# rg2/DeepFluoroLabeling-IPCAI2020

Hardware: AMD Instinct MI355X
Metric: train images/sec, paper U-Net (depth 6, wf 5, BN, strided-conv down, seg + 14-landmark heads), 1x192x192 (8x-downsampled 184x184 padded) (higher is better)
Workload: dtype bf16 (bf16 activations, activation gradients and GEMM weight copies in HBM; bf16 MFMA, fp32 accumulate, BatchNorm statistics, losses, weight gradients and master weights); 1 GPU; BASELINE configs[1]: 8x-downsampled, seg + 14-landmark heat-map dual head, batch 16 per GPU, Dice+NCC loss, SGD nesterov; global_batch=16, image=1x192x192, parallelism=dp1, math=bf16s, optimizer=dfl_amd.SGD(momentum 0.9, nesterov, wd 1e-4)

## Files before the change

### deepfluorolabeling-ipcai2020_amd/_native.py

```python
import ctypes as C
import os

from . import _cabi

_HERE = os.path.dirname(os.path.abspath(__file__))
LIB_PATH = os.environ.get('DFL_LIB_OVERRIDE') or os.path.join(_HERE, 'lib', 'libdfl_hip.so')

i32, i64, f32 = C.c_int32, C.c_int64, C.c_float
fp = C.c_void_p

_CONSTANTS, _STRUCTS, _FUNCTIONS = _cabi.load()
globals().update({name[len('DFL_'):]: value for name, value in _CONSTANTS.items()})
globals().update({cls.__name__: cls for cls in _STRUCTS.values()})
EXPORTS = list(_FUNCTIONS)

CONV_CFG_LATENCY = 39

_KIND_OF = {ConvArgs: OP_CONV, WgradArgs: OP_WGRAD, SumPartialsArgs: OP_SUM_PARTIALS, PackArgs: OP_PACK,
            BnFinalizeArgs: OP_BN_FINALIZE, BnEvalArgs: OP_BN_EVAL, ColstatsArgs: OP_COLSTATS,
            BnBwdFinalizeArgs: OP_BN_BWD_FINALIZE, BnReluBwdArgs: OP_BN_RELU_BWD,
            ReducePartialsArgs: OP_REDUCE_PARTIALS, AffineCopyArgs: OP_AFFINE_COPY, HeadFwdArgs: OP_HEAD_FWD,
            HeadBwdArgs: OP_HEAD_BWD, MemsetArgs: OP_MEMSET, ReduceBatchArgs: OP_REDUCE_BATCH, BnLiveArgs: OP_BN_FINALIZE_LIVE, BnBwdLiveArgs: OP_BN_BWD_FINALIZE_LIVE,
            ConvPairArgs: OP_CONV_PAIR}

# ... 170 lines not shown
        n = len(self.structs) - start if count is None else count
        h = C.c_void_p()
        check(lib().dfl_graph_capture(C.addressof(self._ops) + start * C.sizeof(Op), n, stream, C.addressof(h)),
              'dfl_graph_capture')
        return Graph(h.value, self)

    MIN_GRAPH_OPS = 2

    def graph_chunks(self, stream, start=0, count=None):
        n = len(self.structs) - start if count is None else count
        key = (start, n)
        chunks = self._chunks.get(key)
        if chunks is None:
            chunks, i, end = [], start, start + n
            while i < end:
                plain = self.kinds[i] in (OP_RECORD, OP_WAIT) or self.streams[i] != 0 or self.volatile[i]
                j = i + 1
                while j < end and (self.kinds[j] in (OP_RECORD, OP_WAIT) or self.streams[j] != 0 or self.volatile[j]) == plain:
                    j += 1
                if not plain and j - i >= self.MIN_GRAPH_OPS:
                    chunks.append((i, j - i, self.capture(stream, i, j - i)))
                else:
                    chunks.append((i, j - i, None))
                i = j
            self._chunks[key] = chunks
        return chunks

    def run_graphed(self, stream, start=0, count=None):
        if not self.structs:
            return
        for first, cnt, graph in self.graph_chunks(stream, start, count):
            if graph is not None:
                graph.launch(stream)
            else:
                self.run(stream, first, cnt)
# ... 10 lines not shown
```

### deepfluorolabeling-ipcai2020_amd/csrc/api.hip

```cpp
#include <stdlib.h>
#include <string.h>

#include <mutex>
#include <vector>

#include "common.h"

namespace dfl {
static thread_local char g_err[512] = "";

void set_error(const char* fmt, ...) {
  va_list ap;
  va_start(ap, fmt);
  vsnprintf(g_err, sizeof(g_err), fmt, ap);
  va_end(ap);
}
}

namespace dfl {
static std::mutex g_sync_mu;
static hipStream_t g_side[DFL_MAX_SIDE_STREAMS] = {nullptr};
static std::vector<hipEvent_t> g_events;

static hipStream_t pick_stream(int id, hipStream_t main) {
// ... 59 lines not shown
      (int)sizeof(dfl_preproc_projs_args),   (int)sizeof(dfl_preproc_segs_args),
      (int)sizeof(dfl_restore_labels_args), (int)sizeof(dfl_sim_prepare_args),  (int)sizeof(dfl_sim_gradncc_args),
      (int)sizeof(dfl_expose_args),     (int)sizeof(dfl_sim_patch_prepare_args), (int)sizeof(dfl_sim_patch_gradncc_args),
      (int)sizeof(dfl_raster_mesh),    (int)sizeof(dfl_raster_args),
      (int)sizeof(dfl_sim_gradncc_bwd_args), (int)sizeof(dfl_sim_patch_weights_args), (int)sizeof(dfl_sim_patch_eval_args),
      (int)sizeof(dfl_drr_pose_grad_args),
      (int)sizeof(dfl_sim_bank_gradncc_args), (int)sizeof(dfl_sim_bank_gradncc_bwd_args), (int)sizeof(dfl_sim_patch_bank_gradncc_args),
      (int)sizeof(dfl_drr_object),     (int)sizeof(dfl_drr_args),
      (int)sizeof(dfl_optim_pack_args)};
  if (which < 0 || which >= (int)(sizeof(sizes) / sizeof(sizes[0]))) return -1;
  return sizes[which];
}

static int exec_one(const dfl_op* ops, int i, dfl_stream_t stream, bool serial);

extern "C" int dfl_exec(const dfl_op* ops, int32_t n_ops, dfl_stream_t stream) {
  if (ops == nullptr || n_ops < 0) {
    dfl::set_error("dfl_exec: bad arguments");
    return DFL_ERR_INVALID_ARG;
  }
  for (int i = 0; i < n_ops; ++i) {
    int rc = exec_one(ops, i, stream, false);
    if (rc != DFL_OK) return rc;
  }
  return DFL_OK;
}

extern "C" int dfl_exec_timed(const dfl_op* ops, int32_t n_ops, dfl_stream_t stream, float* ms_out) {
  if (ops == nullptr || n_ops <= 0 || ms_out == nullptr) {
    dfl::set_error("dfl_exec_timed: bad arguments");
    return DFL_ERR_INVALID_ARG;
  }
  hipStream_t s = static_cast<hipStream_t>(stream);
  hipEvent_t* ev = new hipEvent_t[n_ops + 1];
  for (int i = 0; i <= n_ops; ++i) (void)hipEventCreate(&ev[i]);
  int rc = DFL_OK;
  (void)hipEventRecord(ev[0], s);
  int done = 0;
  for (int i = 0; i < n_ops; ++i) {
    rc = exec_one(ops, i, stream, true);
// ... 25 lines not shown
  }
  *graph_out = nullptr;
  (void)stream;
  hipStream_t s = nullptr;
  hipError_t err = hipStreamCreateWithFlags(&s, hipStreamNonBlocking);
  if (err != hipSuccess) {
    dfl::set_error("dfl_graph_capture: hipStreamCreateWithFlags: %s", hipGetErrorString(err));
    return DFL_ERR_LAUNCH;
  }
  err = hipStreamBeginCapture(s, hipStreamCaptureModeThreadLocal);
  if (err != hipSuccess) {
    (void)hipStreamDestroy(s);
    dfl::set_error("dfl_graph_capture: hipStreamBeginCapture: %s", hipGetErrorString(err));
    return DFL_ERR_LAUNCH;
  }
  int rc = DFL_OK;
  for (int i = 0; i < n_ops && rc == DFL_OK; ++i) rc = exec_one(ops, i, static_cast<dfl_stream_t>(s), true);
  hipGraph_t g = nullptr;
  err = hipStreamEndCapture(s, &g);
  (void)hipStreamDestroy(s);
  if (rc != DFL_OK) {
    if (g != nullptr) (void)hipGraphDestroy(g);
    return rc;
  }
  if (err != hipSuccess || g == nullptr) {
    dfl::set_error("dfl_graph_capture: hipStreamEndCapture: %s", hipGetErrorString(err));
    return DFL_ERR_LAUNCH;
  }
  hipGraphExec_t e = nullptr;
  err = hipGraphInstantiate(&e, g, nullptr, nullptr, 0);
  if (err != hipSuccess) {
    (void)hipGraphDestroy(g);
// ... 140 lines not shown
```

### deepfluorolabeling-ipcai2020_amd/plan.py

```python
import ctypes as C
import os

import numpy as np
import torch

from . import _native as nat
from ._native import (ConvArgs, WgradArgs, PackJob, BnFinalizeArgs, ColstatsArgs, BnBwdFinalizeArgs, BnReluBwdArgs,
                      AffineCopyArgs, PoolArgs, HeadFwdArgs, HeadBwdArgs, PackArgs, BnEvalArgs, UpsampleArgs, BnLiveJob, BnLiveArgs,
                      BnBwdLiveJob, BnBwdLiveArgs, MemsetArgs, ReduceJob, ReduceBatchArgs, Program)

BN_EPS = 1.0e-5
BN_MOMENTUM = 0.1


class Act:
    __slots__ = ('t', 'ptr', 'ld', 'N', 'H', 'W', 'C', 'esz')

    def __init__(self, t, ptr, ld, N, H, W, C, esz=4):
        self.t, self.ptr, self.ld, self.N, self.H, self.W, self.C, self.esz = t, ptr, ld, N, H, W, C, esz

    @property
    def M(self):
        return self.N * self.H * self.W

    @property
    def bf16(self):
        return int(self.esz == 2)

    def chan_slice(self, c0, c):
        return Act(self.t, self.ptr + self.esz * c0, self.ld, self.N, self.H, self.W, c, self.esz)


class PlanError(RuntimeError):
    pass


KEEP_GRADS = False


class _Layer:
    __slots__ = ('w', 'wname', 'relu', 'inp', 'gin', 'inp_aff', 'r', 'bn', 'live_bwd')

    def __init__(self, w, wname, relu, inp, gin, inp_aff, r, bn, live_bwd):
        self.w, self.wname, self.relu, self.inp, self.gin, self.inp_aff = w, wname, relu, inp, gin, inp_aff
        self.r, self.bn, self.live_bwd = r, bn, live_bwd


class _Block:
    __slots__ = ('prefix', 'xin', 'out', 'convs', 'rw', 'last_r', 'last_live')
# ... 2 lines not shown
        self.prefix, self.xin, self.out = prefix, xin, out
        self.convs = []
        self.rw = None
        self.last_r = None
        self.last_live = False


class UNetPlan:
    PACK_TILED = os.environ.get('DFL_PACK_TILED', '1') != '0'
    FUSE_BRB = os.environ.get('DFL_FUSE_BRB', '1') != '0'
    FUSE_DOWN_STATS = os.environ.get('DFL_FUSE_DOWN_STATS', '1') != '0'
    FLUSH_BYTES = int(float(os.environ.get('DFL_FLUSH_MB', '16')) * (1 << 20))
    DPRE_OUT_BYTES = int(float(os.environ.get('DFL_DPRE_OUT_MB', '12')) * (1 << 20))
    LIVE_BN = os.environ.get('DFL_LIVE_BN', '1') != '0'
    LIVE_HEAD = os.environ.get('DFL_LIVE_HEAD', '1') != '0'
    BN_R = nat.BN_R

    def __init__(self, cfg, params, buffers, N, H, W, training, need_grad, device, input_grad=False):
        self.cfg = cfg
        self.P = params
        self.Bf = buffers
        self.N, self.H, self.W = N, H, W
        self.training = training
        self.need_grad = need_grad
        self.input_grad = bool(input_grad and need_grad)
        self.dx_in = None
        self.dev = device
        self.lib = nat.lib()
        self._keep = []
        self.fwd = Program()
# ... 8 lines not shown
        self._red_bytes = 0
        self._red_flushes = []
        self.partial_sum_bytes = 0
        self._tiled_host = self._tiled_index = None
        self.math = self.lib.dfl_get_math_mode()
        self.bf16 = self.math == 4
        self.adt = torch.bfloat16 if self.bf16 else torch.float32
        self.aesz = 2 if self.bf16 else 4
        self._packed_split = {}
        self.relu_out = {}
        self._tot_fwd, self._tot_bwd, self._live_jobs, self._live_bwd_pending = [None, 0], [None, 0], [], []
        self.dbg = {}
        self.keep_grads = bool(KEEP_GRADS)
        self.pool_in = {}
        self._latency_form = int(not training and not need_grad and os.environ.get('DFL_PLAN_LATENCY_FORM', '1') != '0')
        self._build()

    def _new(self, nelem, dtype=torch.float32):
        t = torch.empty(max(int(nelem), 1), dtype=dtype, device=self.dev)
        self._keep.append(t)
        return t

    def _const(self, n, value):
        key = ('const', int(n), float(value))
        t = self._scratch.get(key)
        if t is None:
            t = torch.full((int(n),), float(value), dtype=torch.float32, device=self.dev)
            self._keep.append(t)
            self._scratch[key] = t
        return t

    def _act(self, N, H, W, C):
        t = self._new(N * H * W * C, self.adt)
        return Act(t, t.data_ptr(), C, N, H, W, C, self.aesz)

    def _scratch_act(self, key, N, H, W, C):
        need = N * H * W * C
        t = self._scratch.get(key)
        if t is None or t.numel() < need:
            raise PlanError('scratch %s not sized' % key)
        if self.keep_grads:
            return self._act(N, H, W, C)
        return Act(t, t.data_ptr(), C, N, H, W, C, self.aesz)

    def _pack(self, w, kind, flip=0):
        A, B, KH, KW = w.shape
        Cc = KH * KW
        K = {1: Cc * B, 2: Cc * A, 3: A}[kind]
        N = {1: A, 2: B, 3: Cc * B}[kind]
        cin = B if kind == 1 else A
        if self.bf16 and cin % 16 == 0:
            dst = self._new((K + 15) // 16 * N * 16, torch.bfloat16)
            self._packed_split[dst.data_ptr()] = 2
            self._pack_jobs.append((w, dst, A, B, Cc, kind, flip, 2))
            return dst
        dst = self._new((K + 3) // 4 * N * 4)
        split = int(self.math in (1, 3) and cin % 16 == 0)
        self._packed_split[dst.data_ptr()] = split
# ... 11 lines not shown

    def _pack_convT_fwd(self, w):
        return self._pack(w, 3)

    def _pack_convT_dgrad(self, w):
        return self._pack(w, 1)

    @staticmethod
    def _set_pack_job(a, job):
        src, dst, A, B, Cc, kind, flip, split = job
        a.src, a.dst, a.A, a.B, a.C, a.kind, a.flip, a.split = src.data_ptr(), dst.data_ptr(), A, B, Cc, kind, flip, split

    def _upload(self, arr):
        t = torch.from_numpy(np.frombuffer(bytes(arr), dtype=np.uint8).copy()).to(self.dev)
        self._keep.append(t)
        return t.data_ptr()

    def _finish_pack(self):
        self.pack = Program()
        self.pack.extend(self._prep)
        if not self._pack_jobs:
            return
        if self.PACK_TILED:
            self._finish_pack_tiled()
        else:
            self._add_pack_launch(self._pack_jobs)

    def _add_pack_launch(self, jobs):
        arr = (PackJob * len(jobs))()
        for a, job in zip(arr, jobs):
            self._set_pack_job(a, job)
# ... 82 lines not shown
            a.splits = sp
            a.partial = self._shared_scratch('conv_partial', sp * M * Ntot).data_ptr()
        partials = None
        if stat_totals is not None:
            a.stat_totals = stat_totals
            if stat_other is not None:
                a.stat_other, a.ldso = stat_other.ptr, stat_other.ld
            partials = ('live', stat_totals)
        elif stats:
            gm = nat.check(self.lib.dfl_conv_grid_m(C.addressof(a)), 'dfl_conv_grid_m')
            partials = self._new(gm * 2 * Ntot)
            a.stat_partials = partials.data_ptr()
            if stat_other is not None:
                a.stat_other, a.ldso = stat_other.ptr, stat_other.ld
            partials = (partials, 4 * gm if scatter else gm)
        prog.add(a)
        return partials

    def _wgrad(self, prog, g, d, dw, KH, KW, stride, pad, Hout, Wout, in_aff=None, d_split=0, brb=None,
               bias_out=None, bias_plain=False):
        a = WgradArgs()
        a.d_split = d_split
        a.g_bf16, a.d_bf16 = g.bf16, d.bf16
        a.g, a.d, a.dw = g.ptr, d.ptr, dw.data_ptr()
        if in_aff is not None:
            a.in_scale, a.in_shift = in_aff[0].data_ptr(), in_aff[1].data_ptr()
        a.N, a.Hin, a.Win, a.Cg, a.ldg = g.N, g.H, g.W, g.C, g.ld
        a.KH, a.KW, a.stride, a.pad = KH, KW, stride, pad
        a.Hout, a.Wout, a.Cm, a.ldd = Hout, Wout, d.C, d.ld
        if brb is not None:
            r_act, coef = brb
# ... 4 lines not shown
            else:
                a.coef = nat.ptr(coef)
        a.splits = 1
        s = nat.check(self.lib.dfl_wgrad_suggest_splits(C.addressof(a)), 'dfl_wgrad_suggest_splits')
        a.splits = s
        bias_job = None
        if (brb is not None or bias_plain) and bias_out is not None:
            bpart = self._new(s * d.C)
            a.bias_partial = bpart.data_ptr()
            bias_job = (bpart.data_ptr(), bias_out.data_ptr(), d.C, d.C, s, 1)
        n = d.C * g.C * KH * KW
        if s > 1:
            big = 4 * n >= self.FLUSH_BYTES
            part = self._shared_scratch('wg_partial', s * n) if big else self._new(s * n)
            a.partial = part.data_ptr()
        prog.add(a)
        if bias_job is not None:
            self._red_pending.append(bias_job)
            self._red_bytes += 4 * d.C
        if s > 1:
            self._defer_sum(prog, part.data_ptr(), dw.data_ptr(), n, n, s, KH * KW)

    def _defer_sum(self, prog, src, dst, n, stride, count, T=1):
        self._red_pending.append((src, dst, n, stride, count, T))
        self._red_bytes += 4 * n
        self._maybe_flush(prog)

    def _maybe_flush(self, prog):
        if self._red_bytes >= self.FLUSH_BYTES:
            self._flush_sums(prog)

    def _flush_sums(self, prog):
        self._flush_live_bwd(prog)
        jobs = self._red_pending
        if not jobs:
            return
        arr = (ReduceJob * len(jobs))()
        blocks = 0
        for a, (src, dst, n, stride, count, T) in zip(arr, jobs):
            a.src, a.dst, a.n, a.stride, a.count, a.first_block, a.T = src, dst, n, stride, count, blocks, T
            blocks += nat.check(self.lib.dfl_reduce_job_blocks(n, count), 'dfl_reduce_job_blocks')
        self._red_flushes.append((len(prog.structs), [j[1] for j in jobs]))
        self.partial_sum_bytes += sum(4 * n * count for (_, _, n, _, count, _) in jobs)
        prog.add(ReduceBatchArgs(jobs_dev=self._upload(arr), njobs=len(jobs), total_blocks=blocks))
        self._red_pending, self._red_bytes = [], 0

    def _dz_for(self, g, N, H, W, Cc, fused):
        key = 'dpre0' if fused and g.t is self._scratch.get('dz') else 'dz'
        return self._scratch_act(key, N, H, W, Cc)

    def _bn_totals(self, Cc, bwd=False):
        need = self.BN_R * 2 * Cc
        ar = self._tot_bwd if bwd else self._tot_fwd
        if ar[0] is None:
            ar[0] = self._new(sum(self.chans) * self.bd * 2 * self.BN_R * 2, torch.float64)
        assert ar[1] + need <= ar[0].numel()
        ptr = ar[0].data_ptr() + 8 * ar[1]
        ar[1] += need
        return ptr

    def _flush_live_bwd(self, prog):
        jobs = self._live_bwd_pending
        if not jobs:
            return
        arr = (BnBwdLiveJob * len(jobs))()
        for a, j in zip(arr, jobs):
            a.totals, a.save_mean, a.save_invstd = j['tot'], j['mean'].data_ptr(), j['invstd'].data_ptr()
            a.dgamma, a.dbeta, a.sum_out, a.C = j['dgamma'].data_ptr(), j['dbeta'].data_ptr(), nat.ptr(j['sum_out']), j['C']
        dsts = [j[k].data_ptr() for j in jobs for k in ('dgamma', 'dbeta', 'sum_out') if j[k] is not None]
        self._red_flushes.append((len(prog.structs), dsts))
        prog.add(BnBwdLiveArgs(jobs_dev=self._upload(arr), njobs=len(jobs), max_C=max(j['C'] for j in jobs)))
        self._live_bwd_pending = []

    def _finish_live_bn(self):
        jobs = self._live_jobs
        if not jobs:
            return
        arr = (BnLiveJob * len(jobs))()
        for a, j in zip(arr, jobs):
            a.totals, a.gamma, a.beta = j['totals'], j['gamma'].data_ptr(), j['beta'].data_ptr()
            a.running_mean = self.Bf[j['bname'] + '.running_mean'].data_ptr()
            a.running_var = self.Bf[j['bname'] + '.running_var'].data_ptr()
            a.num_batches_tracked = self.Bf[j['bname'] + '.num_batches_tracked'].data_ptr()
            a.scale, a.shift, a.save_mean, a.save_invstd = (j[k].data_ptr() for k in ('scale', 'shift', 'mean', 'invstd'))
            a.count, a.C, a.eps, a.momentum = j['count'], j['C'], BN_EPS, BN_MOMENTUM
        self.fwd.add(BnLiveArgs(jobs_dev=self._upload(arr), njobs=len(jobs), max_C=max(j['C'] for j in jobs)))
        self.fwd.insert(0, MemsetArgs(ptr=self._tot_fwd[0].data_ptr(), bytes=8 * self._tot_fwd[1]))

    def _shared_scratch(self, key, nelem):
        t = self._scratch.get(key)
        if t is None or t.numel() < nelem:
            t = self._new(nelem)
            self._scratch[key] = t
        return t

    def _colsum(self, prog, a, out):
        nb = self.lib.dfl_rowblock_count(a.M, a.C)
        part = self._new(nb * 2 * a.C)
        prog.add(ColstatsArgs(a=a.ptr, b=None, partials=part.data_ptr(), M=a.M, C=a.C, lda=a.ld, ldb=0, nblocks=nb,
                              bf16=a.bf16))
        self._defer_sum(prog, part.data_ptr(), out.data_ptr(), a.C, 2 * a.C, nb)

    _WRAP = ((-1, 0, 1), (0, 1, None), (0, None, 1))

    def _wrap_regions(self, H, W):
        out = []
        for sy, dy, h in ((H - 1, 0, 1), (0, 1, H), (0, H + 1, 1)):
            for sx, dx, w in ((W - 1, 0, 1), (0, 1, W), (0, W + 1, 1)):
                out.append((sy, sx, dy, dx, h, w))
        return out

    def _wrap_pad(self, prog, x):
        n = x.N * (x.H + 2) * (x.W + 2) * x.C
        t = self._new(n, torch.bfloat16 if x.esz == 2 else torch.float32)
        xp = Act(t, t.data_ptr(), x.C, x.N, x.H + 2, x.W + 2, x.C, x.esz)
        for sy, sx, dy, dx, h, w in self._wrap_regions(x.H, x.W):
            prog.add(AffineCopyArgs(x=x.ptr, y=xp.ptr, N=x.N, H=h, W=w, C=x.C, ldx=x.ld, xH=x.H, xW=x.W, xoy=sy, xox=sx,
                                    ldy=xp.ld, yH=xp.H, yW=xp.W, yoy=dy, yox=dx, bf16=x.bf16))
        return xp

    def _wrap_fold(self, prog, dxp, dx, accumulate=0):
        regs = self._wrap_regions(dx.H, dx.W)
        regs.sort(key=lambda r: 0 if (r[4] == dx.H and r[5] == dx.W) else 1)
        for i, (sy, sx, dy, dx_, h, w) in enumerate(regs):
            prog.add(AffineCopyArgs(x=dxp.ptr, y=dx.ptr, N=dx.N, H=h, W=w, C=dx.C, ldx=dxp.ld, xH=dxp.H, xW=dxp.W, xoy=dy, xox=dx_,
                                    ldy=dx.ld, yH=dx.H, yW=dx.W, yoy=sy, yox=sx, accumulate=(accumulate if i == 0 else 1), bf16=dx.bf16))

    def _framed_grad(self, like):
        n = like.N * (like.H + 2) * (like.W + 2) * like.C
        t = self._new(n, self.adt)
        return Act(t, t.data_ptr(), like.C, like.N, like.H + 2, like.W + 2, like.C, self.aesz)

    def _build(self):
        self._levels()
        self._alloc_buffers()
        self._down_forward()
        self._up_forward()
        self._finish_live_bn()
        self._heads_forward()
        if self.need_grad:
# ... 362 lines not shown
        if mfma_head and live_r is not None:
            tot = self._bn_totals(Fx, bwd=True)
            hb.stat_other, hb.ldso, hb.stat_totals = live_r.ptr, live_r.ld, tot
            live = ('live', tot)
        if fused_head:
            part = self._new(4096 * nat.check(self.lib.dfl_head_wgrad_blocks(M_), 'dfl_head_wgrad_blocks'))
            hb.wg_partial = part.data_ptr()
            hb.dw_seg = gs.data_ptr()
            if nl > 0:
                hb.dw_l1 = g1.data_ptr()
                if w2 is not None:
                    hb.dw_l2 = g2.data_ptr()
        else:
            scratch = self._new(M_ * sld)
            hb.scratch = scratch.data_ptr()
        bwd.add(hb, volatile=True)
        if not fused_head:
            off = [self.lib.dfl_head_scratch_off_for(Fx, NC, nm, nl, k) for k in range(5)]
            sact = lambda o, c: Act(scratch, scratch.data_ptr() + 4 * o, sld, N, H_, W_, c)
            self._wgrad(bwd, sact(off[0], Fx), sact(off[1], NC), gs, 1, 1, 1, 0, H_, W_)
            if nl > 0:
                self._wgrad(bwd, sact(off[0], Fx + NC), sact(off[2], nm), g1, 1, 1, 1, 0, H_, W_)
                if w2 is not None:
                    self._wgrad(bwd, sact(off[3], nm), sact(off[4], nl), g2, 1, 1, 1, 0, H_, W_)
        return hb, dx, live

    def _lands_block_backward(self, dfeat, dfeat_a):
        N, G, bwd, u = self.N, self.G, self.bwd, self.feat
        F, Fh = u.C, dfeat.C
        hl, wl = self.heat_hw
        if self.split_heads:
            dout = dfeat_a
            src_u = dfeat.chan_slice(0, F)
            bwd.add(AffineCopyArgs(x=src_u.ptr, y=dout.ptr, N=N, H=hl, W=wl, C=F, ldx=src_u.ld, xH=hl, xW=wl, ldy=dout.ld,
                                   yH=u.H, yW=u.W, yoy=(u.H - hl) // 2, yox=(u.W - wl) // 2, accumulate=1, bf16=dout.bf16))
        else:
            dout = dfeat.chan_slice(0, F)
        d = dfeat.chan_slice(F, Fh - F)
        for j in reversed(range(len(self.lb_layers))):
            src, dst, wname, bname, gin, ho_, wo_ = self.lb_layers[j]
            self._colsum(bwd, d, G[bname])
            self._wgrad(bwd, gin, d, G[wname], 3, 3, 1, 0 if self.circular else self.pad, ho_, wo_)
            wd = self._pack_conv_dgrad(self.P[wname])
            tgt = dout if j == 0 else self._act(N, src.H, src.W, Fh - F)
            if self.circular:
                dzp = self._framed_grad(src)
                self._conv(bwd, d, wd, dzp, 3, 3, 1, 2, src.C)
                self._wrap_fold(bwd, dzp, tgt, accumulate=1 if j == 0 else 0)
            else:
# ... 10 lines not shown
            Ci = self.chans[i]
            st = self._block_backward(rec['blk'], dout, self.dcat[i], fused_in=sums, dxin_stats=True)
            dy = self.dcat[i].chan_slice(0, Ci)
            uin = rec['u']
            bias_name = rec['name'] + ('.up.1.bias' if self.upsample else '.up.bias')
            if st is not None:
                self._defer_sum(bwd, st[0].data_ptr(), G[bias_name].data_ptr(), Ci, 4 * Ci, st[1])
            else:
                self._colsum(bwd, dy, G[bias_name])
            du = self._act(N, uin.H, uin.W, uin.C)
            self.dbg['du:%d' % j] = du
            consumer = self._up[j - 1]['blk'] if j > 0 else self._down[-1]['blk']
            r_last = consumer.last_r
            if self.upsample:
                dylow = self._act(N, uin.H, uin.W, Ci)
                bwd.add(UpsampleArgs(x=dylow.ptr, y=dy.ptr, N=N, H=uin.H, W=uin.W, C=Ci, ldx=dylow.ld, ldy=dy.ld, bf16=dy.bf16),
                        nat.OP_UPSAMPLE_BWD)
                self._wgrad(bwd, uin, dylow, G[rec['name'] + '.up.1.weight'], 1, 1, 1, 0, uin.H, uin.W)
                sums = self._conv(bwd, dylow, self._pack_conv_dgrad(rec['w']), du, 1, 1, 1, 0, uin.C,
                                  stats=r_last is not None, stat_other=r_last,
                                  stat_totals=self._bn_totals(uin.C, bwd=True) if (r_last is not None and consumer.last_live) else None)
            else:
                self._wgrad(bwd, dy, uin, G[rec['name'] + '.up.weight'], 2, 2, 2, 0, uin.H, uin.W)
                wd = self._pack_convT_dgrad(rec['w'])
                sums = self._conv(bwd, dy, wd, du, 2, 2, 2, 0, uin.C, stats=r_last is not None, stat_other=r_last,
                                  stat_totals=self._bn_totals(uin.C, bwd=True) if (r_last is not None and consumer.last_live) else None)
            dout = du
        return dout, sums

    def _down_backward(self, dout, sums):
        N, G, bwd = self.N, self.G, self.bwd
        dnxt = dnxt_sums = None
        for i in reversed(range(self.depth)):
            rec = self._down[i]
            blk = rec['blk']
            out = blk.out
            Ci = self.chans[i]
            if i != self.depth - 1:
                sums = None
                if self.direct_bridge[i]:
                    dout = self.dcat[i].chan_slice(Ci, Ci)
                else:
                    dout = self._act(N, out.H, out.W, Ci)
                    oy, ox, ch, cw = rec['crop']
                    src = self.dcat[i].chan_slice(Ci, Ci)
                    bwd.add(MemsetArgs(ptr=dout.ptr, bytes=dout.esz * dout.M * Ci))
                    bwd.add(AffineCopyArgs(x=src.ptr, y=dout.ptr, N=N, H=ch, W=cw, C=Ci, ldx=src.ld, xH=ch, xW=cw,
                                           ldy=dout.ld, yH=out.H, yW=out.W, yoy=oy, yox=ox, bf16=src.bf16))
                nxt = rec['nxt']
                if self.cfg['max_pool']:
                    bwd.add_pool(PoolArgs(x=out.ptr, y=dnxt.ptr, dx=dout.ptr, N=N, H=out.H, W=out.W, C=Ci, ldx=out.ld,
                                          ldy=dnxt.ld, lddx=dout.ld, bf16=out.bf16), backward=True)
                else:
                    wname = 'downsample_convs.%d' % i
                    if dnxt_sums is not None:
                        self._defer_sum(bwd, dnxt_sums[0].data_ptr(), G[wname + '.bias'].data_ptr(), Ci, 2 * Ci, dnxt_sums[1])
                    else:
                        self._colsum(bwd, dnxt, G[wname + '.bias'])
                    self._wgrad(bwd, out, dnxt, G[wname + '.weight'], 2, 2, 2, 0, nxt.H, nxt.W)
                    wd = self._pack_down_dgrad(self.P[wname + '.weight'])
                    r_last = blk.last_r
                    want = (self.FUSE_DOWN_STATS and r_last is not None and bool(dout.bf16) and bool(r_last.bf16)
                            and out.H == 2 * nxt.H and out.W == 2 * nxt.W)
                    sums = self._conv(bwd, dnxt, wd, dout, 1, 1, 1, 0, 4 * Ci, accumulate=1, scatter=1,
                                      Hout=out.H, Wout=out.W, stats=want, stat_other=r_last if want else None,
                                      stat_totals=self._bn_totals(Ci, bwd=True) if (want and blk.last_live) else None)
            xin = blk.xin
# ... 29 lines not shown
        r, Cout = cv.r, cv.r.C
        res_bias = G[blk.prefix + '.res_conv1x1.bias'] if (self.do_res and d == self.bd - 1) else None
        if cv.bn is None:
            if res_bias is not None:
                self._colsum(bwd, g, res_bias)
            return None
        gamma, mean, invstd, bname = cv.bn
        if sums is not None and sums[0] == 'live':
            assert cv.live_bwd
            self._live_bwd_pending.append(dict(tot=sums[1], mean=mean, invstd=invstd, dgamma=G[bname + '.weight'],
                                               dbeta=G[bname + '.bias'], C=Cout, sum_out=res_bias))
            return dict(tot=sums[1], gamma=gamma, mean=mean, invstd=invstd, count=r.M)
        if sums is None:
            nb = self.lib.dfl_rowblock_count(r.M, Cout)
            part = self._new(nb * 2 * Cout)
            bwd.add(ColstatsArgs(a=g.ptr, b=r.ptr, partials=part.data_ptr(), M=r.M, C=Cout, lda=g.ld,
                                 ldb=r.ld, nblocks=nb, bf16=r.bf16))
            sums = (part, nb)
        part, prow = sums
        coef = self._new(3 * Cout)
        self.dbg['coef:' + cv.relu] = coef
        bwd.add(BnBwdFinalizeArgs(partials=part.data_ptr(), gamma=gamma.data_ptr(),
                                  save_mean=mean.data_ptr(), save_invstd=invstd.data_ptr(),
                                  dgamma=G[bname + '.weight'].data_ptr(),
                                  dbeta=G[bname + '.bias'].data_ptr(), coef=coef.data_ptr(),
                                  count=r.M if self.training else 0,
                                  nblocks=prow, C=Cout))
        if res_bias is not None:
            self._defer_sum(bwd, part.data_ptr(), res_bias.data_ptr(), Cout, 2 * Cout, prow)
        return coef

    def _layer_backward(self, blk, d, g, coef, dout, dxin, dxin_stats):
        cv, G, bwd, N = blk.convs[d], self.G, self.bwd, self.N
        r, inp, Cout, pad, circ = cv.r, cv.inp, cv.r.C, self.pad, self.circular
        self._dpre_turn ^= 1
        if g.t is self._scratch.get('dpre%d' % self._dpre_turn):
            self._dpre_turn ^= 1
        fuse_brb = self.FUSE_BRB and bool(r.bf16) and bool(inp.bf16) and inp.C % 16 == 0 and g.bf16 == r.bf16
        if (self.FUSE_BRB and bool(r.bf16) and g.bf16 == r.bf16 and not inp.bf16 and inp.C == 1
                and d == 0 and dxin is None and Cout in (8, 16, 32, 64)):
            fuse_brb = True
        brb = (r, coef) if fuse_brb else None
        dsplit = 0
        if fuse_brb:
            dpre = g
        else:
            dpre = self._scratch_act('dpre%d' % self._dpre_turn, N, r.H, r.W, Cout)
            nb = self.lib.dfl_rowblock_count(r.M, Cout)
            bpart = self._new(nb * Cout)
            dsplit = int(self.math in (1, 3) and Cout % 16 == 0 and inp.C % 4 == 0 and inp.C * 9 > 12)
            bwd.add(BnReluBwdArgs(dy=g.ptr, r=r.ptr, coef=nat.ptr(coef), dpre=dpre.ptr,
                                  partials=bpart.data_ptr(), M=r.M, C=Cout, lddy=g.ld, ldr=r.ld, ldo=dpre.ld,
                                  nblocks=nb, split_out=dsplit, bf16=r.bf16))
            self._defer_sum(bwd, bpart.data_ptr(), G[cv.wname + '.bias'].data_ptr(), Cout, Cout, nb)
        dmat = None
        if (fuse_brb and bool(inp.bf16) and not circ and pad == 1 and (d > 0 or dxin is not None)
                and 'dmat' in self._scratch and r.M * Cout * 2 <= self.DPRE_OUT_BYTES):
            dmat = self._scratch_act('dmat', N, r.H, r.W, Cout)
            self.dbg['dmat:' + cv.relu] = dmat
        if dmat is None:
            self._layer_wgrad(cv, dpre, d_split=dsplit, brb=brb)
        sums = None
        if circ and (d > 0 or dxin is not None):
            wd = self._pack_conv_dgrad(cv.w)
            dzp = self._framed_grad(inp)
            self._conv(bwd, dpre, wd, dzp, 3, 3, 1, 2, inp.C, x_split=dsplit, brb=brb)
            if d > 0:
                g = self._dz_for(g, N, inp.H, inp.W, Cout, fuse_brb)
# ... 19 lines not shown
            sums = self._conv(bwd, dpre, wd, dxin, 3, 3, 1, 2 - pad, blk.xin.C,
                              x_split=dsplit, stats=dxin_stats and not self.do_res, brb=brb, x_out=dmat)
            if self.do_res:
                sums = self._conv(bwd, dout, self._pack_conv_dgrad(blk.rw), dxin, 1, 1, 1, 0, blk.xin.C,
                                  accumulate=1, stats=dxin_stats)
        if dmat is not None:
            self._layer_wgrad(cv, dmat, bias_plain=True)
        return g, sums

    def _layer_wgrad(self, cv, d, **kw):
        self._wgrad(self.bwd, cv.gin, d, self.G[cv.wname + '.weight'], 3, 3, 1, 0 if self.circular else self.pad, cv.r.H, cv.r.W,
                    in_aff=cv.inp_aff, bias_out=self.G[cv.wname + '.bias'], **kw)

    def _finish_backward(self):
        self._flush_sums(self.bwd)
        if self._tot_bwd[0] is not None:
            self.bwd.insert(0, MemsetArgs(ptr=self._tot_bwd[0].data_ptr(), bytes=8 * self._tot_bwd[1]))
            self._red_flushes = [(idx + 1, dsts) for idx, dsts in self._red_flushes]

    def _grad_ready_ops(self):
        by_ptr = {self.G[k].data_ptr(): k for k in self.grad_names}
        self.grad_ready_op = {}
        for idx, st in enumerate(self.bwd.structs):
            for field in ('dw', 'dst', 'out', 'dgamma', 'dbeta', 'dw_seg', 'dw_l1', 'dw_l2'):
                name = by_ptr.get(getattr(st, field, None))
                if name is not None:
                    self.grad_ready_op[name] = idx
        for idx, dsts in self._red_flushes:
            for d in dsts:
                name = by_ptr.get(d)
# ... 94 lines not shown
```

Before: 4692 images/sec.

## Fork backward weight-gradient ops onto a side stream with span-based dependency tracking

```diff
diff --git a/deepfluorolabeling-ipcai2020_amd/_native.py b/deepfluorolabeling-ipcai2020_amd/_native.py
--- a/deepfluorolabeling-ipcai2020_amd/_native.py
+++ b/deepfluorolabeling-ipcai2020_amd/_native.py
@@ -208,11 +208,11 @@
         if chunks is None:
             chunks, i, end = [], start, start + n
             while i < end:
-                plain = self.kinds[i] in (OP_RECORD, OP_WAIT) or self.streams[i] != 0 or self.volatile[i]
+                plain = self.volatile[i]
                 j = i + 1
-                while j < end and (self.kinds[j] in (OP_RECORD, OP_WAIT) or self.streams[j] != 0 or self.volatile[j]) == plain:
+                while j < end and self.volatile[j] == plain:
                     j += 1
-                if not plain and j - i >= self.MIN_GRAPH_OPS:
+                if not plain and sum(1 for k in self.kinds[i:j] if k not in (OP_RECORD, OP_WAIT)) >= self.MIN_GRAPH_OPS:
                     chunks.append((i, j - i, self.capture(stream, i, j - i)))
                 else:
                     chunks.append((i, j - i, None))
diff --git a/deepfluorolabeling-ipcai2020_amd/csrc/api.hip b/deepfluorolabeling-ipcai2020_amd/csrc/api.hip
--- a/deepfluorolabeling-ipcai2020_amd/csrc/api.hip
+++ b/deepfluorolabeling-ipcai2020_amd/csrc/api.hip
@@ -97,16 +97,75 @@
 
 static int exec_one(const dfl_op* ops, int i, dfl_stream_t stream, bool serial);
 
+namespace dfl {
+static hipEvent_t g_fork_ev[DFL_MAX_SIDE_STREAMS] = {nullptr};
+static hipEvent_t g_join_ev[DFL_MAX_SIDE_STREAMS] = {nullptr};
+
+static bool range_events(int id) {
+  std::lock_guard<std::mutex> lk(g_sync_mu);
+  if (g_fork_ev[id] == nullptr && hipEventCreateWithFlags(&g_fork_ev[id], hipEventDisableTiming) != hipSuccess) return false;
+  if (g_join_ev[id] == nullptr && hipEventCreateWithFlags(&g_join_ev[id], hipEventDisableTiming) != hipSuccess) return false;
+  return true;
+}
+}
+
+static int exec_range(const dfl_op* ops, int n_ops, hipStream_t main) {
+  bool used[DFL_MAX_SIDE_STREAMS] = {false};
+  std::vector<bool> recorded;
+  int rc = DFL_OK;
+  for (int i = 0; i < n_ops && rc == DFL_OK; ++i) {
+    const int sid = ops[i].stream;
+    if (sid < 0 || sid > DFL_MAX_SIDE_STREAMS) {
+      dfl::set_error("dfl_exec: op %d names stream %d (0..%d)", i, sid, DFL_MAX_SIDE_STREAMS);
+      rc = DFL_ERR_INVALID_ARG;
+      break;
+    }
+    if (sid != 0 && !used[sid - 1]) {
+      hipStream_t side = dfl::pick_stream(sid, main);
+      if (side == nullptr || !dfl::range_events(sid - 1) || hipEventRecord(dfl::g_fork_ev[sid - 1], main) != hipSuccess ||
+          hipStreamWaitEvent(side, dfl::g_fork_ev[sid - 1], 0) != hipSuccess) {
+        dfl::set_error("dfl_exec: cannot fork side stream %d (op %d)", sid, i);
+        rc = DFL_ERR_LAUNCH;
+        break;
+      }
+      used[sid - 1] = true;
+    }
+    if (ops[i].kind == DFL_OP_RECORD || ops[i].kind == DFL_OP_WAIT) {
+      const int ev = ops[i].args != nullptr ? static_cast<const dfl_sync_args*>(ops[i].args)->event : -1;
+      if (ev < 0 || ev >= 65536) {
+        dfl::set_error("dfl_exec: op %d names event %d (0..65535)", i, ev);
+        rc = DFL_ERR_INVALID_ARG;
+        break;
+      }
+      if (ops[i].kind == DFL_OP_RECORD) {
+        if ((int)recorded.size() <= ev) recorded.resize(ev + 1, false);
+        recorded[ev] = true;
+      } else if (ev >= (int)recorded.size() || !recorded[ev]) {
+        continue;
+      }
+    }
+    rc = exec_one(ops, i, static_cast<dfl_stream_t>(main), false);
+  }
+  for (int k = 0; k < DFL_MAX_SIDE_STREAMS; ++k) {
+    if (!used[k]) continue;
+    hipStream_t side = dfl::pick_stream(k + 1, main);
+    if (side == nullptr || hipEventRecord(dfl::g_join_ev[k], side) != hipSuccess ||
+        hipStreamWaitEvent(main, dfl::g_join_ev[k], 0) != hipSuccess) {
+      if (rc == DFL_OK) {
+        dfl::set_error("dfl_exec: cannot join side stream %d", k + 1);
+        rc = DFL_ERR_LAUNCH;
+      }
+    }
+  }
+  return rc;
+}
+
 extern "C" int dfl_exec(const dfl_op* ops, int32_t n_ops, dfl_stream_t stream) {
   if (ops == nullptr || n_ops < 0) {
     dfl::set_error("dfl_exec: bad arguments");
     return DFL_ERR_INVALID_ARG;
   }
-  for (int i = 0; i < n_ops; ++i) {
-    int rc = exec_one(ops, i, stream, false);
-    if (rc != DFL_OK) return rc;
-  }
-  return DFL_OK;
+  return exec_range(ops, n_ops, static_cast<hipStream_t>(stream));
 }
 
 extern "C" int dfl_exec_timed(const dfl_op* ops, int32_t n_ops, dfl_stream_t stream, float* ms_out) {
@@ -162,8 +221,7 @@
     dfl::set_error("dfl_graph_capture: hipStreamBeginCapture: %s", hipGetErrorString(err));
     return DFL_ERR_LAUNCH;
   }
-  int rc = DFL_OK;
-  for (int i = 0; i < n_ops && rc == DFL_OK; ++i) rc = exec_one(ops, i, static_cast<dfl_stream_t>(s), true);
+  int rc = exec_range(ops, n_ops, s);
   hipGraph_t g = nullptr;
   err = hipStreamEndCapture(s, &g);
   (void)hipStreamDestroy(s);
diff --git a/deepfluorolabeling-ipcai2020_amd/hazards.py b/deepfluorolabeling-ipcai2020_amd/hazards.py
--- /dev/null
+++ b/deepfluorolabeling-ipcai2020_amd/hazards.py
@@ -0,0 +1,137 @@
+import ctypes as C
+
+from . import _native as nat
+
+EVERYTHING = None
+
+
+def _rows(ptr, rows, ld, width, esz):
+    if not ptr or rows <= 0 or width <= 0:
+        return None
+    pitch, wb = ld * esz, width * esz
+    return (ptr, ptr + (rows - 1) * pitch + wb, pitch if wb < pitch else 0, wb)
+
+
+def _bytes(ptr, n):
+    return (ptr, ptr + n, 0, n) if ptr and n > 0 else None
+
+
+def spans_meet(a, b):
+    if a[0] >= b[1] or b[0] >= a[1]:
+        return False
+    if a[2] and a[2] == b[2]:
+        off = (a[0] - b[0]) % a[2]
+        return off < b[3] or off + a[3] > a[2]
+    return True
+
+
+def _jobs(struct, job_type, host_jobs):
+    arr = host_jobs.get(struct.jobs_dev) if host_jobs else None
+    if arr is None:
+        return None
+    return [arr[k] for k in range(struct.njobs)]
+
+
+def op_spans(st, kind, host_jobs=None):
+    tot = 8 * nat.BN_R * 2
+    rd, wr = [], []
+    if isinstance(st, nat.MemsetArgs):
+        wr.append(_bytes(st.ptr, st.bytes))
+    elif isinstance(st, nat.ConvArgs):
+        ex, ey = (2 if st.x_bf16 else 4), (2 if st.y_bf16 else 4)
+        pin, pout = st.N * st.Hin * st.Win, st.N * st.Hout * st.Wout
+        cy = st.Ntot // 4 if st.scatter2x2 else st.Ntot
+        rd.append(_rows(st.x, pin, st.ldx, st.Cin, ex))
+        if st.x_mode:
+            rd.append(_rows(st.x2, pin, st.ldx2, st.Cin, ex))
+            rd.append(_bytes(st.in_tot, tot * st.Cin) if st.in_tot else _bytes(st.in_scale, 12 * st.Cin))
+        rd.append(_rows(st.add, pout, st.ldadd, st.Ntot, ey))
+        rd.append(_rows(st.stat_other, pout, st.ldso, cy, ey))
+        y = _rows(st.y, pout, st.ldy, cy, ey)
+        wr.append(y)
+        if st.accumulate:
+            rd.append(y)
+        wr.append(_rows(st.x_out, pin, st.ldxo, st.Cin, 2))
+        if st.splits > 1:
+            wr.append(_bytes(st.partial, 4 * st.splits * (pin if st.scatter2x2 else pout) * st.Ntot))
+        if st.stat_partials:
+            gm = nat.check(nat.lib().dfl_conv_grid_m(C.addressof(st)), 'dfl_conv_grid_m')
+            wr.append(_bytes(st.stat_partials, 4 * gm * 2 * st.Ntot))
+        wr.append(_bytes(st.stat_totals, tot * cy))
+    elif isinstance(st, nat.WgradArgs):
+        eg, ed = (2 if st.g_bf16 else 4), (2 if st.d_bf16 else 4)
+        pin, pout = st.N * st.Hin * st.Win, st.N * st.Hout * st.Wout
+        n = st.Cm * st.Cg * st.KH * st.KW
+        rd.append(_rows(st.g, pin, st.ldg, st.Cg, eg))
+        rd.append(_rows(st.d, pout, st.ldd, st.Cm, ed))
+        if st.d_mode:
+            rd.append(_rows(st.d2, pout, st.ldd2, st.Cm, ed))
+            rd.append(_bytes(st.coef_tot, tot * st.Cm) if st.coef_tot else _bytes(st.coef, 12 * st.Cm))
+        s = max(st.splits, 1)
+        wr.append(_bytes(st.partial, 4 * s * n) if s > 1 else _bytes(st.dw, 4 * n))
+        wr.append(_bytes(st.bias_partial, 4 * s * st.Cm))
+    elif isinstance(st, nat.ReduceBatchArgs):
+        jobs = _jobs(st, nat.ReduceJob, host_jobs)
+        if jobs is None:
+            return EVERYTHING
+        for j in jobs:
+            rd.append(_bytes(j.src, 4 * ((j.count - 1) * j.stride + j.n)))
+            wr.append(_bytes(j.dst, 4 * j.n))
+    elif isinstance(st, nat.BnBwdLiveArgs):
+        jobs = _jobs(st, nat.BnBwdLiveJob, host_jobs)
+        if jobs is None:
+            return EVERYTHING
+        for j in jobs:
+            rd += [_bytes(j.totals, tot * j.C), _bytes(j.save_mean, 4 * j.C), _bytes(j.save_invstd, 4 * j.C)]
+            wr += [_bytes(j.dgamma, 4 * j.C), _bytes(j.dbeta, 4 * j.C), _bytes(j.sum_out, 4 * j.C)]
+    elif isinstance(st, nat.ColstatsArgs):
+        e = 2 if st.bf16 else 4
+        rd += [_rows(st.a, st.M, st.lda, st.C, e), _rows(st.b, st.M, st.ldb, st.C, e)]
+        wr.append(_bytes(st.partials, 4 * st.nblocks * 2 * st.C))
+    elif isinstance(st, nat.BnBwdFinalizeArgs):
+        rd.append(_bytes(st.partials, 4 * st.nblocks * 2 * st.C))
+        wr += [_bytes(st.dgamma, 4 * st.C), _bytes(st.dbeta, 4 * st.C), _bytes(st.coef, 12 * st.C)]
+    elif isinstance(st, nat.BnReluBwdArgs):
+        e = 2 if st.bf16 else 4
+        rd += [_rows(st.dy, st.M, st.lddy, st.C, e), _rows(st.r, st.M, st.ldr, st.C, e), _bytes(st.coef, 12 * st.C)]
+        wr += [_rows(st.dpre, st.M, st.ldo, st.C, e), _bytes(st.partials, 4 * st.nblocks * st.C)]
+    else:
+        return EVERYTHING
+    return [s for s in rd if s is not None], [s for s in wr if s is not None]
+
+
+def _conflict(a, b):
+    if a is EVERYTHING or b is EVERYTHING:
+        return True
+    (ra, wa), (rb, wb) = a, b
+    return (any(spans_meet(x, y) for x in wa for y in rb + wb) or any(spans_meet(x, y) for x in ra for y in wb))
+
+
+def unordered_conflicts(prog, start=0, count=None, spans=None, host_jobs=None, n_streams=nat.MAX_SIDE_STREAMS + 1):
+    end = len(prog) if count is None else start + count
+    clock = [[0] * n_streams for _ in range(n_streams)]
+    used = [False] * n_streams
+    events = {}
+    ops = []
+    for i in range(start, end):
+        s, kind, st = prog.streams[i], prog.kinds[i], prog.structs[i]
+        if s != 0 and not used[s]:
+            used[s] = True
+            clock[s] = [max(a, b) for a, b in zip(clock[s], clock[0])]
+        if kind == nat.OP_RECORD:
+            events[st.event] = list(clock[s])
+        elif kind == nat.OP_WAIT:
+            if st.event in events:
+                clock[s] = [max(a, b) for a, b in zip(clock[s], events[st.event])]
+        else:
+            clock[s][s] += 1
+            sp = spans[i] if spans is not None and i in spans else op_spans(st, kind, host_jobs)
+            ops.append((i, s, list(clock[s]), sp))
+    bad = []
+    for b in range(len(ops)):
+        j, sj, cj, spj = ops[b]
+        for a in range(b):
+            i, si, ci, spi = ops[a]
+            if si != sj and cj[si] < ci[si] and _conflict(spi, spj):
+                bad.append((i, j))
+    return bad
diff --git a/deepfluorolabeling-ipcai2020_amd/plan.py b/deepfluorolabeling-ipcai2020_amd/plan.py
--- a/deepfluorolabeling-ipcai2020_amd/plan.py
+++ b/deepfluorolabeling-ipcai2020_amd/plan.py
@@ -33,6 +33,61 @@
 
 class PlanError(RuntimeError):
     pass
+
+
+def _span(a):
+    pitch, width = a.ld * a.esz, a.C * a.esz
+    return (a.ptr, a.ptr + (a.M - 1) * pitch + width, pitch if width < pitch else 0, width)
+
+
+def _flat(ptr, nbytes):
+    return (int(ptr), int(ptr) + int(nbytes), 0, int(nbytes))
+
+
+def _spans_meet(a, b):
+    if a[0] >= b[1] or b[0] >= a[1]:
+        return False
+    if a[2] and a[2] == b[2]:
+        off = (a[0] - b[0]) % a[2]
+        return off < b[3] or off + a[3] > a[2]
+    return True
+
+
+class _Fork:
+    BRANCH = 1
+
+    def __init__(self, prog):
+        self.prog = prog
+        self.pending = []
+        self.events = 0
+        self.at_main = None
+        self.seen = 0
+        self.waits = 0
+
+    def main(self, reads, writes):
+        hit = -1
+        for k, (_, r, w) in enumerate(self.pending):
+            if reads is None or any(_spans_meet(x, y) for x in writes for y in r + w) or any(_spans_meet(x, y) for x in reads for y in w):
+                hit = k
+        if hit >= 0:
+            self.prog.wait(self.pending[hit][0], 0)
+            self.waits += 1
+            del self.pending[:hit + 1]
+        self.at_main = None
+        self.seen += 1
+
+    def fork(self):
+        if self.at_main is None:
+            self.at_main = self.events
+            self.events += 1
+            self.prog.record(self.at_main, 0)
+            self.prog.wait(self.at_main, self.BRANCH)
+        self.seen += 1
+
+    def forked(self, reads, writes):
+        self.prog.record(self.events, self.BRANCH)
+        self.pending.append((self.events, list(reads), list(writes)))
+        self.events += 1
 
 
 KEEP_GRADS = False
@@ -65,6 +120,8 @@
     DPRE_OUT_BYTES = int(float(os.environ.get('DFL_DPRE_OUT_MB', '12')) * (1 << 20))
     LIVE_BN = os.environ.get('DFL_LIVE_BN', '1') != '0'
     LIVE_HEAD = os.environ.get('DFL_LIVE_HEAD', '1') != '0'
+    FORK = os.environ.get('DFL_FORK', '1') != '0'
+    FORK_RING = max(1, int(os.environ.get('DFL_FORK_RING', '2')))
     BN_R = nat.BN_R
 
     def __init__(self, cfg, params, buffers, N, H, W, training, need_grad, device, input_grad=False):
@@ -103,6 +160,9 @@
         self.keep_grads = bool(KEEP_GRADS)
         self.pool_in = {}
         self._latency_form = int(not training and not need_grad and os.environ.get('DFL_PLAN_LATENCY_FORM', '1') != '0')
+        self._deps = _Fork(self.bwd) if (self.FORK and need_grad) else None
+        self._rings = {}
+        self.host_jobs = {}
         self._build()
 
     def _new(self, nelem, dtype=torch.float32):
@@ -130,7 +190,16 @@
             raise PlanError('scratch %s not sized' % key)
         if self.keep_grads:
             return self._act(N, H, W, C)
+        if self._deps is not None:
+            ring = self._rings.setdefault(key, [[t], 0])
+            if len(ring[0]) < self.FORK_RING and ring[1] >= len(ring[0]):
+                ring[0].append(self._new(t.numel(), t.dtype))
+            t = ring[0][ring[1] % len(ring[0])]
+            ring[1] = (ring[1] + 1) % self.FORK_RING
         return Act(t, t.data_ptr(), C, N, H, W, C, self.aesz)
+
+    def _is_scratch(self, t, key):
+        return t is self._scratch.get(key) or any(t is s for s in self._rings.get(key, [[]])[0])
 
     def _pack(self, w, kind, flip=0):
         A, B, KH, KW = w.shape
@@ -172,7 +241,24 @@
     def _upload(self, arr):
         t = torch.from_numpy(np.frombuffer(bytes(arr), dtype=np.uint8).copy()).to(self.dev)
         self._keep.append(t)
+        self.host_jobs[t.data_ptr()] = arr
         return t.data_ptr()
+
+    def _emit(self, prog, a, reads=None, writes=None, branch=False, **kw):
+        dep = self._deps if prog is self.bwd else None
+        if dep is None:
+            prog.add(a, **kw)
+        elif branch:
+            assert reads is not None and writes is not None, 'a branch op declares what it touches'
+            dep.fork()
+            prog.add(a, stream=dep.BRANCH, **kw)
+            idx = len(prog) - 1
+            dep.forked(reads or [], writes or [])
+            return idx
+        else:
+            dep.main(reads, writes)
+            prog.add(a, **kw)
+        return len(prog) - 1
 
     def _finish_pack(self):
         self.pack = Program()
@@ -285,7 +371,20 @@
             if stat_other is not None:
                 a.stat_other, a.ldso = stat_other.ptr, stat_other.ld
             partials = (partials, 4 * gm if scatter else gm)
-        prog.add(a)
+        if prog is self.bwd and self._deps is not None:
+            reads = [_span(t) for t in (x, add, stat_other, brb[0] if brb is not None else None) if t is not None]
+            if accumulate:
+                reads.append(_span(y))
+            writes = [_span(y)] + ([_span(x_out)] if (brb is not None and x_out is not None) else [])
+            if a.partial:
+                writes.append(_flat(a.partial, 4 * a.splits * x.N * (x.H * x.W if scatter else a.Hout * a.Wout) * Ntot))
+            if a.stat_partials:
+                writes.append(_flat(a.stat_partials, 4 * partials[0].numel()))
+            if a.stat_totals:
+                writes.append(_flat(a.stat_totals, 8 * self.BN_R * 2 * (Ntot // 4 if scatter else Ntot)))
+            self._emit(prog, a, reads, writes)
+        else:
+            prog.add(a)
         return partials
 
     def _wgrad(self, prog, g, d, dw, KH, KW, stride, pad, Hout, Wout, in_aff=None, d_split=0, brb=None,
@@ -320,7 +419,20 @@
             big = 4 * n >= self.FLUSH_BYTES
             part = self._shared_scratch('wg_partial', s * n) if big else self._new(s * n)
             a.partial = part.data_ptr()
-        prog.add(a)
+        if prog is self.bwd and self._deps is not None:
+            reads = [_span(g), _flat(d.t.data_ptr(), d.t.numel() * d.t.element_size()) if d_split else _span(d)]
+            if brb is not None:
+                reads.append(_span(brb[0]))
+                if isinstance(brb[1], dict):
+                    reads.append(_flat(brb[1]['tot'], 8 * self.BN_R * 2 * d.C))
+                elif brb[1] is not None:
+                    reads.append(_flat(brb[1].data_ptr(), 4 * brb[1].numel()))
+            writes = [_flat(a.partial, 4 * s * n) if s > 1 else _flat(a.dw, 4 * n)]
+            if a.bias_partial:
+                writes.append(_flat(a.bias_partial, 4 * s * d.C))
+            self._emit(prog, a, reads, writes, branch=True)
+        else:
+            prog.add(a)
         if bias_job is not None:
             self._red_pending.append(bias_job)
             self._red_bytes += 4 * d.C
@@ -346,13 +458,15 @@
         for a, (src, dst, n, stride, count, T) in zip(arr, jobs):
             a.src, a.dst, a.n, a.stride, a.count, a.first_block, a.T = src, dst, n, stride, count, blocks, T
             blocks += nat.check(self.lib.dfl_reduce_job_blocks(n, count), 'dfl_reduce_job_blocks')
-        self._red_flushes.append((len(prog.structs), [j[1] for j in jobs]))
         self.partial_sum_bytes += sum(4 * n * count for (_, _, n, _, count, _) in jobs)
-        prog.add(ReduceBatchArgs(jobs_dev=self._upload(arr), njobs=len(jobs), total_blocks=blocks))
+        idx = self._emit(prog, ReduceBatchArgs(jobs_dev=self._upload(arr), njobs=len(jobs), total_blocks=blocks),
+                         [_flat(src, 4 * ((count - 1) * stride + n)) for (src, _, n, stride, count, _) in jobs],
+                         [_flat(dst, 4 * n) for (_, dst, n, _, _, _) in jobs], branch=True)
+        self._red_flushes.append((idx, [j[1] for j in jobs]))
         self._red_pending, self._red_bytes = [], 0
 
     def _dz_for(self, g, N, H, W, Cc, fused):
-        key = 'dpre0' if fused and g.t is self._scratch.get('dz') else 'dz'
+        key = 'dpre0' if fused and self._is_scratch(g.t, 'dz') else 'dz'
         return self._scratch_act(key, N, H, W, Cc)
 
     def _bn_totals(self, Cc, bwd=False):
@@ -374,8 +488,12 @@
             a.totals, a.save_mean, a.save_invstd = j['tot'], j['mean'].data_ptr(), j['invstd'].data_ptr()
             a.dgamma, a.dbeta, a.sum_out, a.C = j['dgamma'].data_ptr(), j['dbeta'].data_ptr(), nat.ptr(j['sum_out']), j['C']
         dsts = [j[k].data_ptr() for j in jobs for k in ('dgamma', 'dbeta', 'sum_out') if j[k] is not None]
-        self._red_flushes.append((len(prog.structs), dsts))
-        prog.add(BnBwdLiveArgs(jobs_dev=self._upload(arr), njobs=len(jobs), max_C=max(j['C'] for j in jobs)))
+        reads = [_flat(j['tot'], 8 * self.BN_R * 2 * j['C']) for j in jobs]
+        reads += [_flat(j[k].data_ptr(), 4 * j['C']) for j in jobs for k in ('mean', 'invstd')]
+        idx = self._emit(prog, BnBwdLiveArgs(jobs_dev=self._upload(arr), njobs=len(jobs), max_C=max(j['C'] for j in jobs)),
+                         reads, [_flat(j[k].data_ptr(), 4 * j['C']) for j in jobs for k in ('dgamma', 'dbeta', 'sum_out') if j[k] is not None],
+                         branch=True)
+        self._red_flushes.append((idx, dsts))
         self._live_bwd_pending = []
 
     def _finish_live_bn(self):
@@ -403,8 +521,8 @@
     def _colsum(self, prog, a, out):
         nb = self.lib.dfl_rowblock_count(a.M, a.C)
         part = self._new(nb * 2 * a.C)
-        prog.add(ColstatsArgs(a=a.ptr, b=None, partials=part.data_ptr(), M=a.M, C=a.C, lda=a.ld, ldb=0, nblocks=nb,
-                              bf16=a.bf16))
+        self._emit(prog, ColstatsArgs(a=a.ptr, b=None, partials=part.data_ptr(), M=a.M, C=a.C, lda=a.ld, ldb=0, nblocks=nb,
+                                        bf16=a.bf16), [_span(a)], [_flat(part.data_ptr(), 4 * part.numel())])
         self._defer_sum(prog, part.data_ptr(), out.data_ptr(), a.C, 2 * a.C, nb)
 
     _WRAP = ((-1, 0, 1), (0, 1, None), (0, None, 1))
@@ -421,7 +539,7 @@
         t = self._new(n, torch.bfloat16 if x.esz == 2 else torch.float32)
         xp = Act(t, t.data_ptr(), x.C, x.N, x.H + 2, x.W + 2, x.C, x.esz)
         for sy, sx, dy, dx, h, w in self._wrap_regions(x.H, x.W):
-            prog.add(AffineCopyArgs(x=x.ptr, y=xp.ptr, N=x.N, H=h, W=w, C=x.C, ldx=x.ld, xH=x.H, xW=x.W, xoy=sy, xox=sx,
+            self._emit(prog, AffineCopyArgs(x=x.ptr, y=xp.ptr, N=x.N, H=h, W=w, C=x.C, ldx=x.ld, xH=x.H, xW=x.W, xoy=sy, xox=sx,
                                     ldy=xp.ld, yH=xp.H, yW=xp.W, yoy=dy, yox=dx, bf16=x.bf16))
         return xp
 
@@ -429,7 +547,7 @@
         regs = self._wrap_regions(dx.H, dx.W)
         regs.sort(key=lambda r: 0 if (r[4] == dx.H and r[5] == dx.W) else 1)
         for i, (sy, sx, dy, dx_, h, w) in enumerate(regs):
-            prog.add(AffineCopyArgs(x=dxp.ptr, y=dx.ptr, N=dx.N, H=h, W=w, C=dx.C, ldx=dxp.ld, xH=dxp.H, xW=dxp.W, xoy=dy, xox=dx_,
+            self._emit(prog, AffineCopyArgs(x=dxp.ptr, y=dx.ptr, N=dx.N, H=h, W=w, C=dx.C, ldx=dxp.ld, xH=dxp.H, xW=dxp.W, xoy=dy, xox=dx_,
                                     ldy=dx.ld, yH=dx.H, yW=dx.W, yoy=sy, yox=sx, accumulate=(accumulate if i == 0 else 1), bf16=dx.bf16))
 
     def _framed_grad(self, like):
@@ -822,7 +940,7 @@
         else:
             scratch = self._new(M_ * sld)
             hb.scratch = scratch.data_ptr()
-        bwd.add(hb, volatile=True)
+        self._emit(bwd, hb, volatile=True)
         if not fused_head:
             off = [self.lib.dfl_head_scratch_off_for(Fx, NC, nm, nl, k) for k in range(5)]
             sact = lambda o, c: Act(scratch, scratch.data_ptr() + 4 * o, sld, N, H_, W_, c)
@@ -840,7 +958,7 @@
         if self.split_heads:
             dout = dfeat_a
             src_u = dfeat.chan_slice(0, F)
-            bwd.add(AffineCopyArgs(x=src_u.ptr, y=dout.ptr, N=N, H=hl, W=wl, C=F, ldx=src_u.ld, xH=hl, xW=wl, ldy=dout.ld,
+            self._emit(bwd, AffineCopyArgs(x=src_u.ptr, y=dout.ptr, N=N, H=hl, W=wl, C=F, ldx=src_u.ld, xH=hl, xW=wl, ldy=dout.ld,
                                    yH=u.H, yW=u.W, yoy=(u.H - hl) // 2, yox=(u.W - wl) // 2, accumulate=1, bf16=dout.bf16))
         else:
             dout = dfeat.chan_slice(0, F)
@@ -881,8 +999,8 @@
             r_last = consumer.last_r
             if self.upsample:
                 dylow = self._act(N, uin.H, uin.W, Ci)
-                bwd.add(UpsampleArgs(x=dylow.ptr, y=dy.ptr, N=N, H=uin.H, W=uin.W, C=Ci, ldx=dylow.ld, ldy=dy.ld, bf16=dy.bf16),
-                        nat.OP_UPSAMPLE_BWD)
+                self._emit(bwd, UpsampleArgs(x=dylow.ptr, y=dy.ptr, N=N, H=uin.H, W=uin.W, C=Ci, ldx=dylow.ld, ldy=dy.ld, bf16=dy.bf16),
+                           kind=nat.OP_UPSAMPLE_BWD)
                 self._wgrad(bwd, uin, dylow, G[rec['name'] + '.up.1.weight'], 1, 1, 1, 0, uin.H, uin.W)
                 sums = self._conv(bwd, dylow, self._pack_conv_dgrad(rec['w']), du, 1, 1, 1, 0, uin.C,
                                   stats=r_last is not None, stat_other=r_last,
@@ -911,13 +1029,13 @@
                     dout = self._act(N, out.H, out.W, Ci)
                     oy, ox, ch, cw = rec['crop']
                     src = self.dcat[i].chan_slice(Ci, Ci)
-                    bwd.add(MemsetArgs(ptr=dout.ptr, bytes=dout.esz * dout.M * Ci))
-                    bwd.add(AffineCopyArgs(x=src.ptr, y=dout.ptr, N=N, H=ch, W=cw, C=Ci, ldx=src.ld, xH=ch, xW=cw,
+                    self._emit(bwd, MemsetArgs(ptr=dout.ptr, bytes=dout.esz * dout.M * Ci))
+                    self._emit(bwd, AffineCopyArgs(x=src.ptr, y=dout.ptr, N=N, H=ch, W=cw, C=Ci, ldx=src.ld, xH=ch, xW=cw,
                                            ldy=dout.ld, yH=out.H, yW=out.W, yoy=oy, yox=ox, bf16=src.bf16))
                 nxt = rec['nxt']
                 if self.cfg['max_pool']:
-                    bwd.add_pool(PoolArgs(x=out.ptr, y=dnxt.ptr, dx=dout.ptr, N=N, H=out.H, W=out.W, C=Ci, ldx=out.ld,
-                                          ldy=dnxt.ld, lddx=dout.ld, bf16=out.bf16), backward=True)
+                    self._emit(bwd, PoolArgs(x=out.ptr, y=dnxt.ptr, dx=dout.ptr, N=N, H=out.H, W=out.W, C=Ci, ldx=out.ld,
+                                             ldy=dnxt.ld, lddx=dout.ld, bf16=out.bf16), kind=nat.OP_POOL_BWD)
                 else:
                     wname = 'downsample_convs.%d' % i
                     if dnxt_sums is not None:
@@ -977,18 +1095,21 @@
         if sums is None:
             nb = self.lib.dfl_rowblock_count(r.M, Cout)
             part = self._new(nb * 2 * Cout)
-            bwd.add(ColstatsArgs(a=g.ptr, b=r.ptr, partials=part.data_ptr(), M=r.M, C=Cout, lda=g.ld,
-                                 ldb=r.ld, nblocks=nb, bf16=r.bf16))
+            self._emit(bwd, ColstatsArgs(a=g.ptr, b=r.ptr, partials=part.data_ptr(), M=r.M, C=Cout, lda=g.ld,
+                                         ldb=r.ld, nblocks=nb, bf16=r.bf16),
+                       [_span(g), _span(r)], [_flat(part.data_ptr(), 4 * part.numel())])
             sums = (part, nb)
         part, prow = sums
         coef = self._new(3 * Cout)
         self.dbg['coef:' + cv.relu] = coef
-        bwd.add(BnBwdFinalizeArgs(partials=part.data_ptr(), gamma=gamma.data_ptr(),
+        self._emit(bwd, BnBwdFinalizeArgs(partials=part.data_ptr(), gamma=gamma.data_ptr(),
                                   save_mean=mean.data_ptr(), save_invstd=invstd.data_ptr(),
                                   dgamma=G[bname + '.weight'].data_ptr(),
                                   dbeta=G[bname + '.bias'].data_ptr(), coef=coef.data_ptr(),
                                   count=r.M if self.training else 0,
-                                  nblocks=prow, C=Cout))
+                                  nblocks=prow, C=Cout),
+                   [_flat(part.data_ptr(), 4 * part.numel())],
+                   [_flat(coef.data_ptr(), 12 * Cout), _flat(G[bname + '.weight'].data_ptr(), 4 * Cout), _flat(G[bname + '.bias'].data_ptr(), 4 * Cout)])
         if res_bias is not None:
             self._defer_sum(bwd, part.data_ptr(), res_bias.data_ptr(), Cout, 2 * Cout, prow)
         return coef
@@ -997,7 +1118,7 @@
         cv, G, bwd, N = blk.convs[d], self.G, self.bwd, self.N
         r, inp, Cout, pad, circ = cv.r, cv.inp, cv.r.C, self.pad, self.circular
         self._dpre_turn ^= 1
-        if g.t is self._scratch.get('dpre%d' % self._dpre_turn):
+        if self._is_scratch(g.t, 'dpre%d' % self._dpre_turn):
             self._dpre_turn ^= 1
         fuse_brb = self.FUSE_BRB and bool(r.bf16) and bool(inp.bf16) and inp.C % 16 == 0 and g.bf16 == r.bf16
         if (self.FUSE_BRB and bool(r.bf16) and g.bf16 == r.bf16 and not inp.bf16 and inp.C == 1
@@ -1012,9 +1133,12 @@
             nb = self.lib.dfl_rowblock_count(r.M, Cout)
             bpart = self._new(nb * Cout)
             dsplit = int(self.math in (1, 3) and Cout % 16 == 0 and inp.C % 4 == 0 and inp.C * 9 > 12)
-            bwd.add(BnReluBwdArgs(dy=g.ptr, r=r.ptr, coef=nat.ptr(coef), dpre=dpre.ptr,
+            self._emit(bwd, BnReluBwdArgs(dy=g.ptr, r=r.ptr, coef=nat.ptr(coef), dpre=dpre.ptr,
                                   partials=bpart.data_ptr(), M=r.M, C=Cout, lddy=g.ld, ldr=r.ld, ldo=dpre.ld,
-                                  nblocks=nb, split_out=dsplit, bf16=r.bf16))
+                                  nblocks=nb, split_out=dsplit, bf16=r.bf16),
+                       [_span(g), _span(r)] + ([_flat(coef.data_ptr(), 12 * Cout)] if coef is not None else []),
+                       [_flat(dpre.t.data_ptr(), dpre.t.numel() * dpre.t.element_size()) if dsplit else _span(dpre),
+                        _flat(bpart.data_ptr(), 4 * bpart.numel())])
             self._defer_sum(bwd, bpart.data_ptr(), G[cv.wname + '.bias'].data_ptr(), Cout, Cout, nb)
         dmat = None
         if (fuse_brb and bool(inp.bf16) and not circ and pad == 1 and (d > 0 or dxin is not None)
@@ -1064,6 +1188,9 @@
 
     def _finish_backward(self):
         self._flush_sums(self.bwd)
+        if self._deps is not None:
+            if self._deps.seen != sum(1 for k in self.bwd.kinds if k not in (nat.OP_RECORD, nat.OP_WAIT)):
+                raise PlanError('internal: a backward op was recorded past the dependency tracker')
         if self._tot_bwd[0] is not None:
             self.bwd.insert(0, MemsetArgs(ptr=self._tot_bwd[0].data_ptr(), bytes=8 * self._tot_bwd[1]))
             self._red_flushes = [(idx + 1, dsts) for idx, dsts in self._red_flushes]
```

After: 4867 images/sec, median of 6. 3.7% higher.
